# tkoolen/Parametron.jl

Measured on AMD Instinct MI355X. Metric: QP re-evaluations/sec (Q,q,C,d rebuild) at n=4096, higher is better.
Workload: dtype f64; 1 GPU; C2 dense least-squares QP: n=4096 vars, A 4096x4096, m=512 equality rows, fp64; canonical Q,q,const + C,d MOI triplets; n=4096, r=4096, m=512, objective_mode=canonical, instances_per_gpu=1, parallelism=single GPU, replay=tape

## Files before the change

### parametron.jl_amd/csrc/gram_mid.hip

```cpp
#include "affine_tile.h"
#include "gram_common.h"

#ifndef PMT_MID_WPS
#define PMT_MID_WPS 1
#endif
#ifndef PMT_MID_G
#define PMT_MID_G 256
#endif
#ifndef PMT_MID_MAXWG
#define PMT_MID_MAXWG 2304
#endif
#ifndef PMT_MID_D
#define PMT_MID_D 2
#endif
#ifndef PMT_MID_GROUP_US
#define PMT_MID_GROUP_US 1.15
#endif
#ifndef PMT_MID_TAIL_US
#define PMT_MID_TAIL_US 0.95
#endif
#ifndef PMT_MID_SB
#define PMT_MID_SB 8
#endif
#ifndef PMT_MID_FB
#define PMT_MID_FB 4
#endif
#ifndef PMT_MID_FORMAL
#if defined(__HIP_DEVICE_COMPILE__) && !defined(__gfx950__) && !defined(__gfx942__)
#define PMT_MID_FORMAL 1
#else
#define PMT_MID_FORMAL 0
#endif
#endif

#ifdef PMT_MID_TRACE
__device__ unsigned long long g_mid_trace[1024 * 8];
__device__ unsigned long long g_mid_walk[1024 * 8];
__device__ unsigned long long g_mid_riders[1024 * 2];
#define MID_TRACE_WORDS 8
__device__ __forceinline__ void mid_walk_note(unsigned long long *w, int k, unsigned long long t) {
    if (k == 0) { if (w[0]) w[4] += t - w[7]; else w[5] = t; w[0] += 1; }
    else if (k == 1) w[1] += t - w[7];
    else if (k == 3 || k == 5) { w[2] += t - w[7]; w[6] = t; }
    else if (k == 6) { w[3] += t - w[7]; w[6] = t; }
    else return;
    w[7] = t;
}
#define MID_STAMP(k) do { if (threadIdx.x == 0 && blockIdx.x < 1024) { const unsigned long long t_ = wall_clock64(); g_mid_trace[blockIdx.x * 8 + (k)] = t_; \
                          mid_walk_note(reinterpret_cast<unsigned long long *>(sh + MSH), (k), t_); } } while (0)
extern "C" int pmt_mid_trace_read(unsigned long long *host) {
    return hipMemcpyFromSymbol(host, HIP_SYMBOL(g_mid_trace), sizeof(unsigned long long) * 1024 * 8) == hipSuccess ? 0 : 1;
}
extern "C" int pmt_mid_walk_read(unsigned long long *host) {
    return hipMemcpyFromSymbol(host, HIP_SYMBOL(g_mid_walk), sizeof(unsigned long long) * 1024 * 8) == hipSuccess ? 0 : 1;
}
extern "C" int pmt_mid_riders_read(unsigned long long *host) {
    return hipMemcpyFromSymbol(host, HIP_SYMBOL(g_mid_riders), sizeof(unsigned long long) * 1024 * 2) == hipSuccess ? 0 : 1;
}
#else
#define MID_STAMP(k) do { } while (0)
#define MID_TRACE_WORDS 0
#endif

namespace pmt {

constexpr int MT = 64;
constexpr int MACC = 64;
constexpr int MPART = MACC * 64;
constexpr int MSTRIDE = MPART + MT + 8;
constexpr int MPITCH = MT + 1;
constexpr int MFG = 8;
constexpr int MCNT = 16;
constexpr int MQBUF = 4 * 2048;
constexpr int MFLAG = MQBUF + 4 * MT;
constexpr int MMAPS = MFLAG + 8;
constexpr int MSH = MMAPS + 2 * MT;

struct MidArgs {
    const double *A; int64_t lda, rows, cols;
    const double *b; int sign;
    const int64_t *xvar; const int64_t *varmap; int moi;
    QT *out_quad; double *out_csc; double alpha; LT *out_lin; double *out_const;
    int nb;
    int n_off, s_off, s_diag;
    int gpc_off, gpc_diag;
    int n_tail, s_tail, gpc_tail;
    double *ws;
    unsigned *counters;
    int xcd;
    int persist, total;
    unsigned *tickets;
    const AffineRider *riders;
    int nriders, rider_tiles;
};

struct MidPlan { int nb, n_off, s_off, s_diag, gpc_off, gpc_diag, n_tail, s_tail, gpc_tail, wgs; };

static double mid_fold_us(int count) { return 0.5 + 2.6 * (double)cdiv(count, PMT_MID_FB); }

static MidPlan mid_plan(int64_t rows, int64_t cols) {
    MidPlan p;
    p.nb = (int)cdiv(cols, MT);
    p.n_off = p.nb * (p.nb - 1) / 2;
    const int ngroups = (int)std::max<int64_t>(1, cdiv(rows, 8));
    const int maxs = std::max(1, ngroups / 4);
    auto sd = [&](int s) { return std::min(maxs, std::max(1, (5 * s + 7) / 8)); };
    int best = 1;
    double best_t = 1e300;
    for (int s = 1; s <= std::min(maxs, 64); ++s) {
        const int64_t wgs = (int64_t)p.n_off * s + (int64_t)p.nb * sd(s);
        if (s > 1 && wgs > PMT_MID_MAXWG) break;
        const double it_off = (double)cdiv(cdiv(ngroups, s), 4), it_diag = 0.69 * (double)cdiv(cdiv(ngroups, sd(s)), 4);
        const double fold = s <= 1 ? 0.0 : s <= MFG ? mid_fold_us(s) : mid_fold_us(MFG) + 1.5 + mid_fold_us((int)cdiv(s, MFG));
        const double t = (double)cdiv(wgs, PMT_MID_G) * (PMT_MID_GROUP_US * (p.n_off ? std::max(it_off, it_diag) : it_diag) + 5.0 + (s > 1 ? 1.0 : 0.0)) +
                         fold * (1.0 + (double)(p.n_off + p.nb) / PMT_MID_G);
        if (t < best_t) { best_t = t; best = s; }
    }
    int s = best;
#ifdef PMT_TUNING
    if (const char *e = getenv("PMT_MID_S")) { const int v = atoi(e); if (v > 0) s = std::min(v, maxs); }
#endif
    int sdiag = sd(s), ntail = 0, stail = 1;
    if (p.n_off + p.nb > PMT_MID_G) {
        auto wg_us = [&](int c, double w) { return PMT_MID_TAIL_US * w * (double)cdiv(cdiv(ngroups, c), 4) + 5.0 + (c > 1 ? 1.0 : 0.0); };
        const int rem = p.n_off % PMT_MID_G;
        int ct = 1;
        double tail_off = 0.0;
        if (rem) {
            tail_off = 1e300;
            for (int c = 1; c <= std::min(maxs, MFG); ++c) {
                const double t = (double)cdiv((int64_t)rem * c, PMT_MID_G) * wg_us(c, 1.0) + (c > 1 ? mid_fold_us(c) : 0.0);
                if (t < tail_off) { tail_off = t; ct = c; }
            }
        }
        const int last = rem ? (int)(((int64_t)rem * ct) % PMT_MID_G) : 0, free_cus = last ? PMT_MID_G - last : 0;
        const double t_last = rem ? wg_us(ct, 1.0) : wg_us(1, 1.0);
        int cd = 1;
        double tail_diag = 1e300;
        for (int c = 1; c <= std::min(maxs, MFG); ++c) {
            const double t_d = wg_us(c, 0.69);
            const int64_t inside = (int64_t)free_cus * (int64_t)(t_last / t_d);
            const int64_t left = std::max<int64_t>(0, (int64_t)p.nb * c - inside);
            const double t = (double)cdiv(left, PMT_MID_G) * t_d + (c > 1 ? mid_fold_us(c) : 0.0);
            if (t < tail_diag) { tail_diag = t; cd = c; }
        }
        const double t1 = (double)(p.n_off / PMT_MID_G) * wg_us(1, 1.0) + tail_off + tail_diag;
        if (s == 1 || t1 * (PMT_MID_GROUP_US / PMT_MID_TAIL_US) < best_t) { s = 1; sdiag = cd; ntail = ct > 1 ? rem : 0; stail = ct > 1 ? ct : 1; }
    }
#ifdef PMT_TUNING
    if (const char *e = getenv("PMT_MID_TAIL")) { if (atoi(e) == 0) { ntail = 0; stail = 1; } }
#endif
    p.gpc_off = (int)cdiv(ngroups, s);
    p.s_off = (int)cdiv(ngroups, p.gpc_off);
    p.gpc_diag = (int)cdiv(ngroups, sdiag);
    p.s_diag = (int)cdiv(ngroups, p.gpc_diag);
    p.n_tail = ntail;
    p.gpc_tail = (int)cdiv(ngroups, stail);
    p.s_tail = ntail ? (int)cdiv(ngroups, p.gpc_tail) : 1;
    if (p.s_tail <= 1) { p.n_tail = 0; p.s_tail = 1; p.gpc_tail = ngroups; }
    p.wgs = (p.n_off - p.n_tail) * p.s_off + p.n_tail * p.s_tail + p.nb * p.s_diag + 1;
    return p;
}

template <bool DIAG, bool FAST>
__device__ __forceinline__ void mid_load(const MidArgs &g, int64_t row0, int lane, int64_t cj0, int64_t ck0, const unsigned (&voff)[DIAG ? 4 : 8],
                                         f64x2 (&buf)[DIAG ? 4 : 8], f64x2 &cb) {
    constexpr int NG = DIAG ? 4 : 8;
    const int lm = lane & 15, lk = lane >> 4;
    if (FAST) {
        const char *base = reinterpret_cast<const char *>(g.A + row0);
#pragma unroll
        for (int t = 0; t < NG; ++t) buf[t] = *reinterpret_cast<const f64x2 *>(base + voff[t]);
        cb.x = 0.0; cb.y = 0.0;
        if (DIAG && g.b) cb = *reinterpret_cast<const f64x2 *>(g.b + row0 + 2 * lk);
        return;
    }
    const int64_t row = row0 + 2 * lk;
    const bool r0 = row < g.rows, r1 = row + 1 < g.rows;
#pragma unroll
    for (int t = 0; t < NG; ++t) {
        const int64_t col = (t < 4 ? cj0 : ck0) + 16 * (t & 3) + lm;
        const bool cv = col < g.cols;
        const bool v0 = cv && r0, v1 = cv && r1;
        const double *p0 = g.A + (v0 ? col * g.lda + row : 0), *p1 = g.A + (v1 ? col * g.lda + row + 1 : 0);
        const double x = *p0, y = *p1;
        buf[t].x = v0 ? x : 0.0;
        buf[t].y = v1 ? y : 0.0;
    }
    cb.x = 0.0; cb.y = 0.0;
    if (DIAG && g.b) {
        const double x = g.b[r0 ? row : 0], y = g.b[r1 ? row + 1 : 0];
        cb.x = r0 ? x : 0.0;
        cb.y = r1 ? y : 0.0;
    }
}

template <bool DIAG>
__device__ __forceinline__ void mid_compute(double *__restrict__ rot, const f64x2 (&buf)[DIAG ? 4 : 8], const f64x2 &cb, int sign, int lane,
                                            double (&acc)[MACC], double (&qacc)[4]) {
    constexpr int BO = DIAG ? 0 : 4;
    const int lm = lane & 15, lrow = lane & 48;
#pragma unroll
    for (int t = 0; t < 4; ++t) *reinterpret_cast<f64x2 *>(rot + (t * 64 + lane) * 2) = buf[BO + t];
    f64x2 bv[4][4];
#pragma unroll
    for (int c = 0; c < 4; ++c) {
        bv[c][0] = buf[BO + c];
#pragma unroll
        for (int r = 1; r < 4; ++r) {
            bv[c][r] = *reinterpret_cast<const f64x2 *>(rot + (c * 64 + lrow + ((lm + 4 * r) & 15)) * 2);
        }
    }
    __builtin_amdgcn_sched_barrier(0);
    constexpr int NC = 4;
#pragma unroll
    for (int c = 0; c < NC; ++c)
#pragma unroll
        for (int tm = 0; tm < (DIAG ? c + 1 : 4); ++tm) {
            const int a = (tm * 4 + c) * 4;
            acc[a] = __builtin_amdgcn_mfma_f64_4x4x4f64(buf[tm].x, bv[c][0].x, acc[a], 0, 0, 0);
        }
#pragma unroll
    for (int c = 0; c < NC; ++c)
#pragma unroll
        for (int tm = 0; tm < (DIAG ? c + 1 : 4); ++tm) {
            const int a = (tm * 4 + c) * 4;
            acc[a] = __builtin_amdgcn_mfma_f64_4x4x4f64(buf[tm].y, bv[c][0].y, acc[a], 0, 0, 0);
        }
    __builtin_amdgcn_sched_barrier(0);
#pragma unroll
    for (int c = 0; c < NC; ++c) {
#pragma unroll
        for (int r = 1; r < 4; ++r)
#pragma unroll
            for (int tm = 0; tm < (DIAG ? c + 1 : 4); ++tm) {
                const int a = (tm * 4 + c) * 4 + r;
                acc[a] = __builtin_amdgcn_mfma_f64_4x4x4f64(buf[tm].x, bv[c][r].x, acc[a], 0, 0, 0);
            }
#pragma unroll
        for (int r = 1; r < 4; ++r)
#pragma unroll
            for (int tm = 0; tm < (DIAG ? c + 1 : 4); ++tm) {
                const int a = (tm * 4 + c) * 4 + r;
                acc[a] = __builtin_amdgcn_mfma_f64_4x4x4f64(buf[tm].y, bv[c][r].y, acc[a], 0, 0, 0);
            }
    }
    if (DIAG) {
        const double c0 = signed_const(cb.x, sign), c1 = signed_const(cb.y, sign);
#pragma unroll
        for (int t = 0; t < 4; ++t) qacc[t] = __builtin_amdgcn_mfma_f64_4x4x4f64(buf[t].x, c0, qacc[t], 0, 0, 0);
#pragma unroll
        for (int t = 0; t < 4; ++t) qacc[t] = __builtin_amdgcn_mfma_f64_4x4x4f64(buf[t].y, c1, qacc[t], 0, 0, 0);
    }
}

#define MID_SB() __builtin_amdgcn_sched_barrier(0)
template <bool DIAG>
__device__ __forceinline__ void mid_step(const MidArgs &g, double *__restrict__ rot, int64_t next_row0, const char *base_a, const char *base_b,
                                         unsigned (&voff)[DIAG ? 4 : 8], f64x2 (&buf)[DIAG ? 4 : 8], f64x2 &cb, int sign, int lane,
                                         double (&acc)[MACC], double (&qacc)[4]) {
    constexpr int BO = DIAG ? 0 : 4;
    const int lm = lane & 15, lrow = lane & 48, lk = lane >> 4;
    auto reload = [&](int t) {
        asm volatile("" : "+v"(voff[t]));
        buf[t] = *reinterpret_cast<const f64x2 *>((t < 4 ? base_a : base_b) + voff[t]);
    };
    f64x2 bv[4][4];
#pragma unroll
    for (int c = 0; c < 4; ++c) bv[c][0] = buf[BO + c];
    auto lds_op = [&](int i) {
        if (i < 4) *reinterpret_cast<f64x2 *>(rot + (i * 64 + lane) * 2) = buf[BO + i];
        else {
            const int c = (i - 4) / 3, r = 1 + (i - 4) % 3;
            bv[c][r] = *reinterpret_cast<const f64x2 *>(rot + (c * 64 + lrow + ((lm + 4 * r) & 15)) * 2);
        }
    };
    MID_SB();
    int k = 0;
#pragma unroll
    for (int pass = 0; pass < 2; ++pass)
#pragma unroll
        for (int c = 0; c < 4; ++c)
#pragma unroll
            for (int tm = 0; tm < (DIAG ? c + 1 : 4); ++tm) {
                const int a = (tm * 4 + c) * 4;
                acc[a] = __builtin_amdgcn_mfma_f64_4x4x4f64(pass ? buf[tm].y : buf[tm].x, pass ? bv[c][0].y : bv[c][0].x, acc[a], 0, 0, 0);
                if (k < 16) { MID_SB(); lds_op(k); MID_SB(); }
                ++k;
            }
    if (DIAG) {
        const double c0 = signed_const(cb.x, sign), c1 = signed_const(cb.y, sign);
#pragma unroll
        for (int t = 0; t < 4; ++t) qacc[t] = __builtin_amdgcn_mfma_f64_4x4x4f64(buf[t].x, c0, qacc[t], 0, 0, 0);
#pragma unroll
        for (int t = 0; t < 4; ++t) qacc[t] = __builtin_amdgcn_mfma_f64_4x4x4f64(buf[t].y, c1, qacc[t], 0, 0, 0);
        MID_SB();
        cb = *reinterpret_cast<const f64x2 *>((g.b ? g.b : g.A) + next_row0 + 2 * lk);
    }
    MID_SB();
    int nb = 0;
#pragma unroll
    for (int tm = 0; tm < 4; ++tm) {
#pragma unroll
        for (int pass = 0; pass < 2; ++pass)
#pragma unroll
            for (int c = (DIAG ? tm : 0); c < 4; ++c)
#pragma unroll
                for (int r = 1; r < 4; ++r) {
                    const int a = (tm * 4 + c) * 4 + r;
                    acc[a] = __builtin_amdgcn_mfma_f64_4x4x4f64(pass ? buf[tm].y : buf[tm].x, pass ? bv[c][r].y : bv[c][r].x, acc[a], 0, 0, 0);
                    if (!DIAG && nb < 4) { MID_SB(); reload(4 + nb); MID_SB(); ++nb; }
                }
        MID_SB();
        reload(tm);
        MID_SB();
    }
}

__host__ __device__ constexpr bool mid_used(bool diag, int a) { return !diag || (a >> 4) <= ((a >> 2) & 3); }

__device__ __forceinline__ void mid_pos(int lane, int a, int &row, int &col) {
    const int i = lane >> 4, b = (lane >> 2) & 3, j = lane & 3;
    row = 16 * (a >> 4) + 4 * b + i;
    col = 16 * ((a >> 2) & 3) + 4 * ((b + (a & 3)) & 3) + j;
}

__device__ __forceinline__ void mid_maps(const MidArgs &g, double *sh, int tid, int jb, int kb) {
    u64 *cmap = reinterpret_cast<u64 *>(sh + MMAPS);
    if (tid >= 2 * MT || (!g.out_quad && jb != kb)) return;
    const int64_t i = (tid < MT ? (int64_t)kb * MT + tid : (int64_t)jb * MT + tid - MT);
    const int64_t v = i < g.cols ? g.xvar[i] : 1;
    cmap[tid] = (u64)(g.moi ? map_var(g.varmap, v) : v);
}

__device__ __forceinline__ void mid_epilogue(const MidArgs &g, double *sh, int tid, int jb, int kb) {
    const int wave = tid >> 6, lane = tid & 63;
    const int64_t n = g.cols, j0 = (int64_t)jb * MT, k0 = (int64_t)kb * MT;
    double *tile = sh;
    const double *qfin = sh + MT * MPITCH;
    const u64 *cmap = reinterpret_cast<const u64 *>(sh + MMAPS);
    const u64 *rmap = cmap + MT;
    if (g.out_csc) {
        const int64_t j = j0 + lane;
#pragma unroll 4
        for (int col = wave; col < MT; col += 4) {
            const int64_t k = k0 + col;
            double c = tile[lane * MPITCH + col];
            if (g.moi || j != k) c = 2 * c;
            if (k < n && j <= k) g.out_csc[k * (k + 1) / 2 + j] = g.alpha * c;
        }
    }
    if (g.out_quad) {
        u64 *out = reinterpret_cast<u64 *>(g.out_quad);
        u64 *desc = reinterpret_cast<u64 *>(sh + MT * MPITCH + MT);
        if (tid < MT) {
            const int64_t j = j0 + tid;
            const int64_t kstart = j > k0 ? j : k0;
            const int64_t kend = (k0 + MT < n) ? k0 + MT : n;
            const int64_t nterms = (j < n && kend > kstart) ? kend - kstart : 0;
            desc[2 * tid] = (u64)(j * n - (j * (j - 1)) / 2 + (kstart - j)) * 3;
            desc[2 * tid + 1] = (u64)nterms | (u64)(kstart - k0) << 16 | (u64)(kstart == j ? 1 : 0) << 24;
        }
        __syncthreads();
        const bool moi = g.moi != 0;
        const int uwave = __builtin_amdgcn_readfirstlane(wave);
#pragma unroll 4
        for (int i = 0; i < MT / 4; ++i) {
            const int row = 4 * i + uwave;
            const u64 w0 = desc[2 * row], info = desc[2 * row + 1];
            const int nterms = (int)(info & 0xffff), coff = (int)((info >> 16) & 0xff);
            const bool dg = ((info >> 24) & 1) != 0;
            double c = tile[row * MPITCH + coff + lane];
            const u64 m = cmap[(coff + lane) & (MT - 1)], rv = rmap[row];
            if (moi || !(dg && lane == 0)) c = 2 * c;
            if (lane < nterms) {
                u64 *d = out + w0 + 3 * lane;
                d[0] = (u64)__double_as_longlong(c);
                d[1] = rv;
                d[2] = m;
            }
        }
    }
    if (jb == kb && tid < MT) {
        const int64_t j = j0 + tid;
        if (j < n) {
            LT t;
            t.coeff = 2 * qfin[tid];
            t.var = (int64_t)rmap[tid];
            g.out_lin[j] = t;
        }
    }
}

__device__ __forceinline__ void mid_constant(const MidArgs &g, double *sh, int tid) {
    const int wave = tid >> 6, lane = tid & 63;
    double s0 = 0.0, s1 = 0.0;
    if (g.b && g.sign) {
        for (int64_t i = tid; i < g.rows; i += 512) { const double c = signed_const(g.b[i], g.sign); s0 = s0 + c * c; }
        for (int64_t i = tid + 256; i < g.rows; i += 512) { const double c = signed_const(g.b[i], g.sign); s1 = s1 + c * c; }
    }
#pragma unroll
    for (int off = 32; off > 0; off >>= 1) { s0 = s0 + __shfl_down(s0, off, 64); s1 = s1 + __shfl_down(s1, off, 64); }
    if (lane == 0) { sh[wave] = s0; sh[4 + wave] = s1; }
    __syncthreads();
    if (tid == 0) {
        double v = sh[0];
#pragma unroll
        for (int w = 1; w < 8; ++w) v = v + sh[w];
        *g.out_const = v;
    }
}

__device__ __forceinline__ void mid_put(double *p, double v) {
#if PMT_MID_FORMAL
    *p = v;
#else
    __hip_atomic_store(p, v, __ATOMIC_RELAXED, __HIP_MEMORY_SCOPE_AGENT);
#endif
}
__device__ __forceinline__ double mid_get(const double *p) {
#if PMT_MID_FORMAL
    return *p;
#else
    return __hip_atomic_load(p, __ATOMIC_RELAXED, __HIP_MEMORY_SCOPE_AGENT);
#endif
}

template <bool DIAG, int W>
__device__ __forceinline__ void mid_tail(const MidArgs &g, double *sh, int lane, double (&acc)[MACC], const double (&qacc)[4], int nchunk, double *w) {
    constexpr int KEEP1 = (W >> 1) * 32, GIVE1 = 32 - KEEP1, KEEP2 = KEEP1 + (W & 1) * 16, GIVE2 = KEEP1 + 16 - (W & 1) * 16;
    double *mine = sh + W * 2048;
    const double *half = sh + (W ^ 2) * 2048, *quarter = sh + (W ^ 1) * 2048;
    const bool qlane = (lane & 3) == 0;
    const int qcol = 4 * ((lane >> 2) & 3) + (lane >> 4);
#pragma unroll
    for (int a = 0; a < 32; a += 2)
        if (mid_used(DIAG, GIVE1 + a)) { f64x2 v; v.x = acc[GIVE1 + a]; v.y = acc[GIVE1 + a + 1]; *reinterpret_cast<f64x2 *>(mine + (a * 32 + lane) * 2) = v; }
    if (DIAG && qlane) {
#pragma unroll
        for (int t = 0; t < 4; ++t) sh[MQBUF + W * MT + 16 * t + qcol] = qacc[t];
    }
    __syncthreads();
#pragma unroll
    for (int a = 0; a < 32; a += 2)
        if (mid_used(DIAG, KEEP1 + a)) {
            const f64x2 v = *reinterpret_cast<const f64x2 *>(half + (a * 32 + lane) * 2);
            acc[KEEP1 + a] = acc[KEEP1 + a] + v.x; acc[KEEP1 + a + 1] = acc[KEEP1 + a + 1] + v.y;
        }
    double qsum = 0.0;
    if (DIAG && W == 0) qsum = (sh[MQBUF + lane] + sh[MQBUF + 2 * MT + lane]) + (sh[MQBUF + MT + lane] + sh[MQBUF + 3 * MT + lane]);
    __syncthreads();
#pragma unroll
    for (int a = 0; a < 16; a += 2)
        if (mid_used(DIAG, GIVE2 + a)) { f64x2 v; v.x = acc[GIVE2 + a]; v.y = acc[GIVE2 + a + 1]; *reinterpret_cast<f64x2 *>(mine + (a * 32 + lane) * 2) = v; }
    __syncthreads();
#pragma unroll
    for (int a = 0; a < 16; a += 2)
        if (mid_used(DIAG, KEEP2 + a)) {
            const f64x2 v = *reinterpret_cast<const f64x2 *>(quarter + (a * 32 + lane) * 2);
            acc[KEEP2 + a] = acc[KEEP2 + a] + v.x; acc[KEEP2 + a + 1] = acc[KEEP2 + a + 1] + v.y;
        }
    __syncthreads();
    if (nchunk == 1) {
#pragma unroll
        for (int a = KEEP2; a < KEEP2 + 16; ++a) {
            if (!mid_used(DIAG, a)) continue;
            int row, col;
            mid_pos(lane, a, row, col);
            sh[row * MPITCH + col] = acc[a];
        }
        if (DIAG && W == 0) sh[MT * MPITCH + lane] = qsum;
        return;
    }
#pragma unroll
    for (int a = KEEP2; a < KEEP2 + 16; ++a) if (mid_used(DIAG, a)) mid_put(&w[a * 64 + lane], acc[a]);
    if (DIAG && W == 0) mid_put(&w[MPART + lane], qsum);
#if PMT_MID_FORMAL
    __builtin_amdgcn_fence(__ATOMIC_RELEASE, "agent");
#else
    __builtin_amdgcn_s_waitcnt(0);
#endif
}

template <bool DIAG>
__device__ __forceinline__ void mid_fold(const double *p, int count, int64_t stride, int tid, double (&sum)[16], double &qs) {
#pragma unroll
    for (int u = 0; u < 16; ++u) sum[u] = 0.0;
    qs = 0.0;
    for (int c0 = 0; c0 < count; c0 += PMT_MID_FB) {
        double v[PMT_MID_FB][16], qv[PMT_MID_FB];
#pragma unroll
        for (int cc = 0; cc < PMT_MID_FB; ++cc) {
            const double *pc = p + (int64_t)min(c0 + cc, count - 1) * stride;
#pragma unroll
            for (int u = 0; u < 16; ++u) {
                const int a = (tid >> 6) + 4 * u;
                v[cc][u] = 0.0;
                if (mid_used(DIAG, a)) v[cc][u] = mid_get(pc + tid + 256 * u);
            }
            qv[cc] = 0.0;
            if (DIAG && tid < MT) qv[cc] = mid_get(pc + MPART + tid);
        }
#pragma unroll
        for (int cc = 0; cc < PMT_MID_FB; ++cc) {
            const bool live = c0 + cc < count;
#pragma unroll
            for (int u = 0; u < 16; ++u) { const double t = sum[u] + v[cc][u]; sum[u] = live ? t : sum[u]; }
            const double t = qs + qv[cc];
            qs = live ? t : qs;
        }
    }
}

struct MidWalk {
    bool early;
    unsigned *ticket; int id0;
    int *slot;
    int drawn;
    bool next_full; int njb, nkb, nrank;
    bool pre;
};

template <int N>
__device__ __forceinline__ void mid_forget(f64x2 (&buf)[PMT_MID_D][N]) {
#pragma unroll
    for (int d = 0; d < PMT_MID_D; ++d)
#pragma unroll
        for (int t = 0; t < N; ++t) asm volatile("" : "=v"(buf[d][t].x), "=v"(buf[d][t].y));
}

template <bool DIAG>
__device__ __forceinline__ auto &mid_buf(f64x2 (&own)[PMT_MID_D][4], f64x2 (&walk)[PMT_MID_D][8]) {
    if constexpr (DIAG) return own; else return walk;
}

template <bool DIAG, bool FAST>
__device__ __forceinline__ void mid_body(const MidArgs &g, double *sh, int tid, int jb, int kb, int chunk, int nchunk, int gpc, int first_wg, unsigned *counter,
                                         MidWalk &wk, f64x2 (&pbuf)[PMT_MID_D][8]) {
    constexpr int NG = DIAG ? 4 : 8;
    constexpr int D = PMT_MID_D;
    asm volatile("" : "+v"(tid));
    const int lane = tid & 63;
    const int wave = __builtin_amdgcn_readfirstlane(tid >> 6);
    const int lm = lane & 15, lk = lane >> 4;
    const int64_t cj0 = (int64_t)jb * MT, ck0 = (int64_t)kb * MT;
    const int ngroups = (int)((g.rows + 7) >> 3);
    const int g0 = chunk * gpc + wave, g1 = min((chunk + 1) * gpc, ngroups);
    const int my = g1 > g0 ? (g1 - g0 + 3) / 4 : 0;
    const bool ragged = FAST && (g.rows & 7) && my > 0 && g0 + 4 * (my - 1) == ngroups - 1;
    const int nfast = ragged ? my - 1 : my;

    MID_STAMP(0);
    mid_maps(g, sh, tid, jb, kb);
    double acc[MACC], qacc[4] = {0.0, 0.0, 0.0, 0.0};
#pragma unroll
    for (int a = 0; a < MACC; ++a) acc[a] = 0.0;
    unsigned voff[NG];
#pragma unroll
    for (int t = 0; t < NG; ++t) voff[t] = (unsigned)((min((t < 4 ? cj0 : ck0) + 16 * (t & 3) + lm, g.cols - 1) * g.lda + 2 * lk) * 8);
    double *rot = sh + wave * 512;
    f64x2 dbuf[D][4], cb[D];
    auto &buf = mid_buf<DIAG>(dbuf, pbuf);
    auto row_of = [&](int s) { return (int64_t)(g0 + 4 * min(s, max(nfast - 1, 0))) * 8; };
    const bool pre = !DIAG && wk.pre;
    bool pf = false;
    if (!DIAG && FAST) pf = wk.early && wk.next_full && nchunk == 1 && !ragged && nfast > 0 && nfast % D == 0 && (int64_t)(kb + 1) * MT <= g.cols;
    const int ahead_at = __builtin_amdgcn_readfirstlane(pf ? nfast - D : -1);
    const int64_t shift_a = pf ? ((int64_t)wk.njb * MT - cj0) * g.lda * 8 : 0, shift_b = pf ? ((int64_t)wk.nkb * MT - ck0) * g.lda * 8 : 0;
    if (nfast > 0) {
        if (!pre) {
#pragma unroll
            for (int d = 0; d < D; ++d) {
                __builtin_amdgcn_sched_barrier(0);
                mid_load<DIAG, FAST>(g, row_of(d), lane, cj0, ck0, voff, buf[d], cb[d]);
            }
            __builtin_amdgcn_sched_barrier(0);
        }
        if (FAST) {
            int s0 = 0;
            for (; s0 + D <= nfast; s0 += D) {
                const bool ahead = s0 == ahead_at;
#pragma unroll
                for (int d = 0; d < D; ++d) {
                    const int64_t row = ahead ? row_of(d) : row_of(s0 + d + D);
                    const char *base = reinterpret_cast<const char *>(g.A + row);
                    mid_step<DIAG>(g, rot, row, base + (ahead ? shift_a : 0), base + (ahead ? shift_b : 0), voff, buf[d], cb[d], g.sign, lane, acc, qacc);
                }
            }
#pragma unroll
            for (int d = 0; d < D - 1; ++d)
                if (s0 + d < nfast) mid_compute<DIAG>(rot, buf[d], cb[d], g.sign, lane, acc, qacc);
        } else {
            for (int s0 = 0; s0 < nfast; s0 += D) {
#pragma unroll
                for (int d = 0; d < D; ++d) {
                    if (s0 + d < nfast) mid_compute<DIAG>(rot, buf[d], cb[d], g.sign, lane, acc, qacc);
                    mid_load<DIAG, FAST>(g, row_of(s0 + d + D), lane, cj0, ck0, voff, buf[d], cb[d]);
                }
            }
        }
    }
    if (ragged) {
        mid_load<DIAG, false>(g, (int64_t)(ngroups - 1) * 8, lane, cj0, ck0, voff, buf[0], cb[0]);
        mid_compute<DIAG>(rot, buf[0], cb[0], g.sign, lane, acc, qacc);
    }

    MID_STAMP(1);
    wk.pre = pf;
    unsigned drawn = 0;
    if (!DIAG && wk.early && tid == 0) drawn = __hip_atomic_fetch_add(wk.ticket, 1u, __ATOMIC_RELAXED, __HIP_MEMORY_SCOPE_AGENT);
    unsigned *flag = reinterpret_cast<unsigned *>(sh + MFLAG);
    double *w = g.ws + (int64_t)(first_wg + chunk) * MSTRIDE;
    __syncthreads();
    if (wave == 0) mid_tail<DIAG, 0>(g, sh, lane, acc, qacc, nchunk, w);
    else if (wave == 1) mid_tail<DIAG, 1>(g, sh, lane, acc, qacc, nchunk, w);
    else if (wave == 2) mid_tail<DIAG, 2>(g, sh, lane, acc, qacc, nchunk, w);
    else mid_tail<DIAG, 3>(g, sh, lane, acc, qacc, nchunk, w);
    MID_STAMP(2);
    if (nchunk > 1) {
        const bool two = nchunk > MFG;
        const int gfirst = two ? (chunk / MFG) * MFG : 0;
        const int n1 = two ? min(MFG, nchunk - gfirst) : nchunk;
        unsigned *c1 = two ? counter + 1 + chunk / MFG : counter;
        __syncthreads();
        if (tid == 0) *flag = __hip_atomic_fetch_add(c1, 1u, __ATOMIC_RELAXED, __HIP_MEMORY_SCOPE_AGENT);
        __syncthreads();
        MID_STAMP(3);
        if (*flag != (unsigned)(n1 - 1)) { mid_forget(buf); return; }
#if PMT_MID_FORMAL
        __builtin_amdgcn_fence(__ATOMIC_ACQUIRE, "agent");
#endif
        if (tid == 0) __hip_atomic_store(c1, 0u, __ATOMIC_RELAXED, __HIP_MEMORY_SCOPE_AGENT);
        double sum[16], qs;
        double *p = g.ws + (int64_t)(first_wg + gfirst) * MSTRIDE;
        mid_fold<DIAG>(p, n1, MSTRIDE, tid, sum, qs);
        if (two) {
#pragma unroll
            for (int u = 0; u < 16; ++u) if (mid_used(DIAG, (tid >> 6) + 4 * u)) mid_put(p + tid + 256 * u, sum[u]);
            if (DIAG && tid < MT) mid_put(p + MPART + tid, qs);
#if PMT_MID_FORMAL
            __builtin_amdgcn_fence(__ATOMIC_RELEASE, "agent");
#else
            __builtin_amdgcn_s_waitcnt(0);
#endif
            __syncthreads();
            if (tid == 0) *flag = __hip_atomic_fetch_add(counter, 1u, __ATOMIC_RELAXED, __HIP_MEMORY_SCOPE_AGENT);
            __syncthreads();
            const int ng = (nchunk + MFG - 1) / MFG;
            if (*flag != (unsigned)(ng - 1)) { mid_forget(buf); return; }
#if PMT_MID_FORMAL
            __builtin_amdgcn_fence(__ATOMIC_ACQUIRE, "agent");
#endif
            if (tid == 0) __hip_atomic_store(counter, 0u, __ATOMIC_RELAXED, __HIP_MEMORY_SCOPE_AGENT);
            mid_fold<DIAG>(g.ws + (int64_t)first_wg * MSTRIDE, ng, (int64_t)MFG * MSTRIDE, tid, sum, qs);
        }
        __syncthreads();
        MID_STAMP(4);
#pragma unroll
        for (int u = 0; u < 16; ++u) {
            const int a = (tid >> 6) + 4 * u;
            if (!mid_used(DIAG, a)) continue;
            int row, col;
            mid_pos(lane, a, row, col);
            sh[row * MPITCH + col] = sum[u];
        }
        if (DIAG && tid < MT) sh[MT * MPITCH + tid] = qs;
        mid_forget(buf);
    }
    if (!DIAG && wk.early && tid == 0) *wk.slot = wk.id0 + 8 * (int)drawn;
    __syncthreads();
    if (!DIAG && wk.early) wk.drawn = *wk.slot;
    MID_STAMP(5);
    mid_epilogue(g, sh, tid, jb, kb);
#ifdef PMT_MID_TRACE
    __builtin_amdgcn_s_waitcnt(0);
    MID_STAMP(6);
#endif
}

__device__ __forceinline__ int mid_xcd_rank(int id, int base, int n) {
    const int x = id & 7, end = base + n;
    int start = 0;
    for (int y = 0; y < x; ++y) {
        const int fy = base + ((y - base) & 7);
        start += fy < end ? ((end - 1 - fy) >> 3) + 1 : 0;
    }
    return start + ((id - (base + ((x - base) & 7))) >> 3);
}

__device__ __forceinline__ void mid_tile_of(int t, int nb, int &jb, int &kb) {
    constexpr int SB = PMT_MID_SB;
    const int nsb = (nb + SB - 1) / SB;
    for (int K = 0; K < nsb; ++K) {
        const int wK = min(SB, nb - SB * K);
        for (int J = 0; J <= K; ++J) {
            const int cnt = J < K ? SB * wK : wK * (wK - 1) / 2;
            if (t >= cnt) { t -= cnt; continue; }
            if (J < K) { jb = SB * J + t / wK; kb = SB * K + t % wK; return; }
            int kk = 1;
            while (t >= kk) { t -= kk; ++kk; }
            jb = SB * K + t; kb = SB * K + kk;
            return;
        }
    }
    jb = 0; kb = 1;
}

struct MidItem { int kind, jb, kb, chunk, nch, gpc, first, rank; };
__device__ __forceinline__ MidItem mid_decode(const MidArgs &g, int id) {
    MidItem it = {2, 0, 0, 0, 1, 0, 0, 0};
    const int nbody = g.n_off - g.n_tail, wbody = nbody * g.s_off, noff = wbody + g.n_tail * g.s_tail;
    if (id < noff) {
        const bool tail = id >= wbody;
        const int base = tail ? wbody : 0, ntile = tail ? g.n_tail : nbody, nch = tail ? g.s_tail : g.s_off;
        const int k = g.xcd ? mid_xcd_rank(id, base, ntile * nch) : ((id - base) % nch) * ntile + (id - base) / nch;
        const int chunk = k / ntile;
        const int rank = (tail ? nbody : 0) + (k - chunk * ntile);
        int t = rank, jb, kb;
        if (g.xcd) mid_tile_of(t, g.nb, jb, kb);
        else {
            kb = 1;
            while (t >= kb) { t -= kb; ++kb; }
            jb = t;
        }
        it.kind = 0; it.jb = jb; it.kb = kb; it.chunk = chunk; it.nch = nch; it.gpc = tail ? g.gpc_tail : g.gpc_off;
        it.first = tail ? wbody + (rank - nbody) * g.s_tail : rank * g.s_off;
        it.rank = rank;
        return it;
    }
    if (id < noff + g.nb * g.s_diag) {
        const int k = g.xcd ? mid_xcd_rank(id, noff, g.nb * g.s_diag) : ((id - noff) % g.s_diag) * g.nb + (id - noff) / g.s_diag;
        const int chunk = k / g.nb, jb = k - chunk * g.nb;
        it.kind = 1; it.jb = jb; it.kb = jb; it.chunk = chunk; it.nch = g.s_diag; it.gpc = g.gpc_diag; it.first = noff + jb * g.s_diag; it.rank = g.n_off + jb;
    }
    return it;
}

template <bool FAST>
__device__ __forceinline__ void mid_item(const MidArgs &g, double *sh, int tid, const MidItem &it, MidWalk &wk, f64x2 (&pbuf)[PMT_MID_D][8]) {
    if (it.kind == 0) {
        mid_body<false, FAST>(g, sh, tid, it.jb, it.kb, it.chunk, it.nch, it.gpc, it.first, g.counters + it.rank * MCNT, wk, pbuf);
        return;
    }
    wk.pre = false;
    if (it.kind == 1) mid_body<true, FAST>(g, sh, tid, it.jb, it.kb, it.chunk, it.nch, it.gpc, it.first, g.counters + it.rank * MCNT, wk, pbuf);
    else mid_constant(g, sh, tid);
    mid_forget(pbuf);
}

__device__ __forceinline__ void mid_rider_tile(const AffineRider &r, int local, double *sh) {
    int t;
    asm volatile("v_mov_b32 %0, %1" : "=v"(t) : "v"((int)threadIdx.x));
    const int by = local / r.tiles_x, bx = local - by * r.tiles_x;
    double *tile = sh;
    u64 *vmx = reinterpret_cast<u64 *>(sh + TILE * PITCH);
#define MID_RIDE(NTV, TRV, NTLV)                                                                                                         \
    affine_tile_body<1, NTV, TRV, NTLV>(r.A, r.lda, r.rows, r.cols, r.xvar, r.b, r.sign, r.varmap, r.row_offset, r.out, r.out_consts,   \
                                        r.vec_in, r.vec_out, bx, by, t, tile, vmx)
    if (r.ntl) { if (r.tr == 32) MID_RIDE(true, 32, true); else MID_RIDE(true, 64, true); }
#ifdef PMT_TUNING
    else if (!r.nt) { if (r.tr == 32) MID_RIDE(false, 32, false); else MID_RIDE(false, 64, false); }
#endif
    else { if (r.tr == 32) MID_RIDE(true, 32, false); else MID_RIDE(true, 64, false); }
#undef MID_RIDE
}
static_assert(TILE * PITCH + TILE <= MQBUF, "a rider's tile and its variable-map row live in the front of the kernel's LDS");

template <bool FAST>
__global__ __launch_bounds__(256, PMT_MID_WPS) void gram_mid_kernel(MidArgs g) {
    __shared__ double sh[MSH + MID_TRACE_WORDS];
    __shared__ int next_id, ahead_id;
    const int tid = threadIdx.x;
    const int x = blockIdx.x & 7, per = gridDim.x >> 3;
#ifdef PMT_MID_TRACE
    if (tid == 0) for (int i = 0; i < MID_TRACE_WORDS; ++i) reinterpret_cast<unsigned long long *>(sh + MSH)[i] = 0;
#endif
    f64x2 pbuf[PMT_MID_D][8];
    MidWalk wk = {};
    wk.ticket = g.tickets + x; wk.id0 = x + 8 * per; wk.slot = &ahead_id;
    const int wbody = (g.n_off - g.n_tail) * g.s_off;
    const bool look = FAST && g.persist && g.s_off == 1;
    int id = blockIdx.x, hand = -1;
    if (look) {
        if (tid == 0) next_id = wk.id0 + 8 * (int)__hip_atomic_fetch_add(wk.ticket, 1u, __ATOMIC_RELAXED, __HIP_MEMORY_SCOPE_AGENT);
        __syncthreads();
        hand = next_id;
    }
    MidItem cur = mid_decode(g, id);
    for (;;) {
        wk.early = hand >= 0 && hand < wbody;
        wk.next_full = false;
        if (wk.early) {
            const MidItem nx = mid_decode(g, hand);
            wk.next_full = (int64_t)(nx.kb + 1) * MT <= g.cols;
            wk.njb = nx.jb; wk.nkb = nx.kb; wk.nrank = nx.rank;
        }
        mid_item<FAST>(g, sh, tid, cur, wk, pbuf);
        if (!g.persist) return;
        __syncthreads();
        if (wk.early) {
            id = hand; hand = wk.drawn;
            cur.jb = wk.njb; cur.kb = wk.nkb; cur.first = cur.rank = wk.nrank;
            continue;
        }
        if (hand >= 0) { id = hand; hand = -1; }
        else {
            if (tid == 0) next_id = wk.id0 + 8 * (int)__hip_atomic_fetch_add(wk.ticket, 1u, __ATOMIC_RELAXED, __HIP_MEMORY_SCOPE_AGENT);
            __syncthreads();
            id = next_id;
        }
        if (id >= g.total) break;
        cur = mid_decode(g, id);
    }
    if (g.rider_tiles > 0) {
        int mine = 0;
        for (;;) {
            __syncthreads();
            if (tid == 0) next_id = (int)__hip_atomic_fetch_add(g.tickets + 9, 1u, __ATOMIC_RELAXED, __HIP_MEMORY_SCOPE_AGENT);
            __syncthreads();
            const int rt = __builtin_amdgcn_readfirstlane(next_id);
            if (rt >= g.rider_tiles) break;
            int k = 0;
            while (k + 1 < g.nriders && rt >= g.riders[k + 1].first_tile) ++k;
            mid_rider_tile(g.riders[k], rt - g.riders[k].first_tile, sh);
            ++mine;
        }
#ifdef PMT_MID_TRACE
        __builtin_amdgcn_s_waitcnt(0);
        if (tid == 0 && blockIdx.x < 1024) { g_mid_riders[blockIdx.x * 2] = (unsigned long long)mine; g_mid_riders[blockIdx.x * 2 + 1] = wall_clock64(); }
#endif
        (void)mine;
    }
#ifdef PMT_MID_TRACE
    if (tid == 0 && blockIdx.x < 1024) {
        for (int i = 0; i < 7; ++i) g_mid_walk[blockIdx.x * 8 + i] = reinterpret_cast<unsigned long long *>(sh + MSH)[i];
        g_mid_walk[blockIdx.x * 8 + 7] = wall_clock64();
    }
#endif
    if (tid == 0) {
        const unsigned gone = __hip_atomic_fetch_add(g.tickets + 8, 1u, __ATOMIC_RELAXED, __HIP_MEMORY_SCOPE_AGENT);
        if (gone == gridDim.x - 1) {
#pragma unroll
            for (int i = 0; i < 10; ++i) __hip_atomic_store(g.tickets + i, 0u, __ATOMIC_RELAXED, __HIP_MEMORY_SCOPE_AGENT);
        }
    }
}

__global__ __launch_bounds__(256) void gram_mid_constant_kernel(MidArgs g) {
    __shared__ double sh[8];
    mid_constant(g, sh, threadIdx.x);
}
int launch_gram_mid_constant(const double *b, int sign, int64_t rows, double *out_const, hipStream_t s) {
    MidArgs g = {};
    g.rows = rows; g.b = (b && sign) ? b : nullptr; g.sign = g.b ? sign : 0; g.out_const = out_const;
    PMT_LAUNCH_NAMED("gram_mid_constant_kernel", gram_mid_constant_kernel, dim3(1), dim3(256), 0, s, g);
    return check_launch("gram_mid_constant_kernel");
}

size_t gram_mid_workspace_bytes(int64_t rows, int64_t cols) {
    if (cols <= 0) return 0;
    const MidPlan p = mid_plan(rows, cols);
    return sizeof(double) * (size_t)p.wgs * MSTRIDE;
}
bool gram_mid_persistent(int64_t rows, int64_t cols) { return cols > 0 && rows > 0 && mid_plan(rows, cols).wgs >= 2 * PMT_MID_G; }
int gram_mid_counters(int64_t cols) { const int nb = (int)cdiv(cols, MT); return MCNT * (nb * (nb + 1) / 2) + 16; }

int launch_gram_mid(const double *A, int64_t lda, int64_t rows, int64_t cols, const int64_t *xvar, const double *b, int sign, int moi,
                    const int64_t *varmap, pmt_quadratic_term *out_quad, double *out_csc, double alpha, pmt_linear_term *out_lin,
                    double *out_const, void *workspace, unsigned *counters, const void *riders, int nriders, int rider_tiles, hipStream_t s) {
    if (!workspace || !counters) return fail(PMT_INVALID_ARGUMENT, "quad_gram: workspace required");
    const MidPlan p = mid_plan(rows, cols);
    MidArgs g;
    g.A = A; g.lda = lda; g.rows = rows; g.cols = cols; g.b = (b && sign) ? b : nullptr; g.sign = g.b ? sign : 0;
    g.xvar = xvar; g.varmap = varmap; g.moi = moi; g.out_quad = reinterpret_cast<QT *>(out_quad); g.out_csc = out_csc; g.alpha = alpha;
    g.out_lin = reinterpret_cast<LT *>(out_lin); g.out_const = out_const;
    g.nb = p.nb; g.n_off = p.n_off; g.s_off = p.s_off; g.s_diag = p.s_diag; g.gpc_off = p.gpc_off; g.gpc_diag = p.gpc_diag;
    g.n_tail = p.n_tail; g.s_tail = p.s_tail; g.gpc_tail = p.gpc_tail;
    g.ws = reinterpret_cast<double *>(workspace); g.counters = counters;
    g.xcd = rows * cols * 8 > ((int64_t)4 << 20);
    const bool fast = (reinterpret_cast<uintptr_t>(A) & 15) == 0 && (lda & 1) == 0 && (reinterpret_cast<uintptr_t>(g.b) & 15) == 0 &&
                      (uint64_t)lda * (uint64_t)cols * 8 < (1ull << 32);
    g.total = p.wgs;
    g.persist = p.wgs >= 2 * PMT_MID_G;
    g.tickets = counters + gram_mid_counters(cols) - 16;
    const bool ride = g.persist && riders && nriders > 0 && rider_tiles > 0;
    g.riders = ride ? static_cast<const AffineRider *>(riders) : nullptr; g.nriders = ride ? nriders : 0; g.rider_tiles = ride ? rider_tiles : 0;
    const unsigned grid = g.persist ? (unsigned)PMT_MID_G : (unsigned)p.wgs;
    if (fast) PMT_LAUNCH_NAMED("gram_mid_kernel", (gram_mid_kernel<true>), dim3(grid), dim3(256), 0, s, g);
    else PMT_LAUNCH_NAMED("gram_mid_kernel", (gram_mid_kernel<false>), dim3(grid), dim3(256), 0, s, g);
    return check_launch("gram_mid_kernel");
}

}
```

Measured before the change: 929.0 re-evaluations/s.

## Restructure quad-triplet epilogue with wave-uniform addressing and 16-byte vector stores

Replaces the shared-memory descriptor table and its barrier with per-wave scalar address recurrences computed from readfirstlane'd block indices. For full off-diagonal tiles, each lane writes interleaved 16-byte chunks of the 24-byte triplets, so stores are contiguous and vectorized. Tile loads are batched MWR rows at a time to raise memory-level parallelism. Diagonal and edge tiles keep a per-row path that now uses readlane for row variables. The cost is more complex index math and more registers, which could lower occupancy.

```diff
diff --git a/parametron.jl_amd/csrc/gram_mid.hip b/parametron.jl_amd/csrc/gram_mid.hip
--- a/parametron.jl_amd/csrc/gram_mid.hip
+++ b/parametron.jl_amd/csrc/gram_mid.hip
@@ -351,33 +351,75 @@
         }
     }
     if (g.out_quad) {
-        u64 *out = reinterpret_cast<u64 *>(g.out_quad);
-        u64 *desc = reinterpret_cast<u64 *>(sh + MT * MPITCH + MT);
-        if (tid < MT) {
-            const int64_t j = j0 + tid;
-            const int64_t kstart = j > k0 ? j : k0;
-            const int64_t kend = (k0 + MT < n) ? k0 + MT : n;
-            const int64_t nterms = (j < n && kend > kstart) ? kend - kstart : 0;
-            desc[2 * tid] = (u64)(j * n - (j * (j - 1)) / 2 + (kstart - j)) * 3;
-            desc[2 * tid + 1] = (u64)nterms | (u64)(kstart - k0) << 16 | (u64)(kstart == j ? 1 : 0) << 24;
-        }
-        __syncthreads();
+        constexpr int MWR = 8;
         const bool moi = g.moi != 0;
         const int uwave = __builtin_amdgcn_readfirstlane(wave);
-#pragma unroll 4
-        for (int i = 0; i < MT / 4; ++i) {
-            const int row = 4 * i + uwave;
-            const u64 w0 = desc[2 * row], info = desc[2 * row + 1];
-            const int nterms = (int)(info & 0xffff), coff = (int)((info >> 16) & 0xff);
-            const bool dg = ((info >> 24) & 1) != 0;
-            double c = tile[row * MPITCH + coff + lane];
-            const u64 m = cmap[(coff + lane) & (MT - 1)], rv = rmap[row];
-            if (moi || !(dg && lane == 0)) c = 2 * c;
-            if (lane < nterms) {
-                u64 *d = out + w0 + 3 * lane;
-                d[0] = (u64)__double_as_longlong(c);
-                d[1] = rv;
-                d[2] = m;
+        const int ujb = __builtin_amdgcn_readfirstlane(jb), ukb = __builtin_amdgcn_readfirstlane(kb);
+        const int64_t uj0 = (int64_t)ujb * MT, uk0 = (int64_t)ukb * MT;
+        const bool dtile = ujb == ukb;
+        const int64_t kend = (uk0 + MT < n) ? uk0 + MT : n;
+        const int64_t jw = uj0 + uwave;
+        int64_t w = 24 * (jw * n - (jw * (jw - 1)) / 2 + (dtile ? 0 : uk0 - jw));
+        int64_t dw = 24 * (4 * n - 4 * jw - (dtile ? 6 : 10));
+        char *out = reinterpret_cast<char *>(g.out_quad);
+        const u64 rmine = rmap[lane];
+        auto row_var = [&](int row) {
+            const unsigned lo = (unsigned)__builtin_amdgcn_readlane((int)(unsigned)rmine, row), hi = (unsigned)__builtin_amdgcn_readlane((int)(rmine >> 32), row);
+            return (u64)hi << 32 | lo;
+        };
+        if (ujb < ukb && uk0 + MT <= n && uj0 + MT <= n) {
+            typedef u64 u64x2u __attribute__((ext_vector_type(2), aligned(8)));
+#pragma unroll
+            for (int h = 0; h < 2; ++h) {
+                if (h == 1 && lane >= 32) break;
+                const int q = lane + 64 * h, m = q / 3, cls = q - 3 * m;
+                const bool is0 = cls == 0, is1 = cls == 1;
+                const u64 cv = cmap[2 * m + (cls == 2 ? 1 : 0)];
+                const double *tcol = tile + uwave * MPITCH + 2 * m + (cls == 0 ? 0 : 1);
+                int64_t wr = w, dwr = dw;
+#pragma unroll
+                for (int i0 = 0; i0 < MT / 4; i0 += MWR) {
+                    double c[MWR];
+                    u64 rv[MWR];
+#pragma unroll
+                    for (int r = 0; r < MWR; ++r) { c[r] = tcol[4 * (i0 + r) * MPITCH]; rv[r] = rmap[4 * (i0 + r) + uwave]; }
+#pragma unroll
+                    for (int r = 0; r < MWR; ++r) {
+                        const u64 c2 = (u64)__double_as_longlong(2 * c[r]);
+                        u64x2u v;
+                        v.x = is0 ? c2 : (is1 ? cv : rv[r]);
+                        v.y = is0 ? rv[r] : (is1 ? c2 : cv);
+                        *reinterpret_cast<u64x2u *>(out + wr + (unsigned)(16 * q)) = v;
+                        wr += dwr; dwr -= 24 * 16;
+                    }
+                }
+            }
+        } else {
+#pragma unroll
+            for (int i0 = 0; i0 < MT / 4; i0 += MWR / 2) {
+                double c[MWR / 2];
+                u64 m[MWR / 2];
+#pragma unroll
+                for (int r = 0; r < MWR / 2; ++r) {
+                    const int row = 4 * (i0 + r) + uwave, coff = dtile ? row : 0;
+                    c[r] = tile[row * MPITCH + coff + lane];
+                    m[r] = cmap[(coff + lane) & (MT - 1)];
+                }
+#pragma unroll
+                for (int r = 0; r < MWR / 2; ++r) {
+                    const int row = 4 * (i0 + r) + uwave;
+                    const int64_t j = uj0 + row, kstart = dtile ? j : uk0;
+                    const int nterms = (j < n && kend > kstart) ? (int)(kend - kstart) : 0;
+                    const double v = (moi || !(dtile && lane == 0)) ? 2 * c[r] : c[r];
+                    const u64 rv = row_var(row);
+                    if (lane < nterms) {
+                        u64 *d = reinterpret_cast<u64 *>(out + w + (unsigned)(24 * lane));
+                        d[0] = (u64)__double_as_longlong(v);
+                        d[1] = rv;
+                        d[2] = m[r];
+                    }
+                    w += dw; dw -= 24 * 16;
+                }
             }
         }
     }
```

Result: no change. 935.2 re-evaluations/s, median of 6 (+0.7%).
